# danijar/crafter

Hardware: AMD Instinct MI355X
Metric: env-steps/sec (whole node), random policy, 4096 envs (higher is better)
Workload: dtype u8/i32 (+f64 render filters)

## Files before the change

### __graft_entry__.py

```python
import pathlib
import sys

ROOT = pathlib.Path(__file__).resolve().parent
if str(ROOT) not in sys.path:
  sys.path.insert(0, str(ROOT))


def build():
  from crafter_amd import build as hip_build
  path = hip_build.build()
  print(f'[build] {path}')
  from oracle import noise
  print(f'[build] {noise.build()}')
  from tests.hostsim import build as hostsim_build
  print(f'[build] {hostsim_build.build()}')
  from tests.hostsim import symbolic_build
  print(f'[build] {symbolic_build.build()}')
  from tests.hostsim import final_build
  print(f'[build] {final_build.build()}')
  from tests.hostsim import levels_build
  print(f'[build] {levels_build.build()}')
  from tests.hostsim import subset_build
  print(f'[build] {subset_build.build()}')
  import crafter_amd
  from crafter_amd import lib
  lib.load()
  print('[build] crafter_amd imported, libcrafter_hip.so loaded, ABI', lib.load().crafter_abi_version())


def smoke():
  import numpy as np
  import torch
  from crafter_amd import BatchedEnv
  from oracle.crafter_oracle import OracleEnv
  from tests.parity import assert_same
  assert torch.cuda.is_available(), 'smoke() needs a GPU'
  seeds = [1000, 1001, 1002, 1003]
  env = BatchedEnv(len(seeds), seeds=seeds, device='cuda:0', auto_reset=False, semantic=True)
  orcs = [OracleEnv(seed=s) for s in seeds]
  obs = env.reset().cpu().numpy()
  for i, o in enumerate(orcs):
    assert np.array_equal(obs[i], o.reset()), f'reset obs env {i}'
  rs = np.random.RandomState(0)
  for t in range(30):
    acts = rs.randint(0, 17, size=len(seeds)).astype(np.int32)
    obs, rew, done, info = env.step(torch.from_numpy(acts).to('cuda:0'))
    obs, rew, done = obs.cpu().numpy(), rew.cpu().numpy(), done.cpu().numpy()
    for i, o in enumerate(orcs):
      ob, r, d, _ = o.step(int(acts[i]))
      assert np.array_equal(obs[i], ob) and rew[i] == np.float32(r) and bool(done[i]) == bool(d), (t, i)
  for i, o in enumerate(orcs):
    assert_same(env.snapshot(i), o.snapshot(), f'smoke env {i}')
  env.check_errors()
  print(f'[smoke] ok: {len(seeds)} envs x 30 steps bit-exact vs oracle on {torch.cuda.get_device_name(0)}; '
        f'LDS/env {env.lds_bytes} B')

# ... 6 lines not shown
```

### crafter_amd/build.py

```python
import pathlib
import shutil
import subprocess

ROOT = pathlib.Path(__file__).resolve().parent
SRC = ROOT / 'csrc' / 'crafter_hip.hip'
SRC_ROLLOUT = ROOT / 'csrc' / 'crafter_rollout.hip'
SRC_SUBSET = ROOT / 'csrc' / 'crafter_subset.hip'
OUT = ROOT / '_lib' / 'libcrafter_hip.so'
FLAGS = ['--offload-arch=gfx950', '-O3', '-std=c++17', '-ffp-contract=off', '-fPIC', '-shared']
CFLAGS = [f for f in FLAGS if f != '-shared']
ROLLOUT_FLAGS = ['-mllvm', '-disable-machine-licm']


def sources():
  return ([SRC, SRC_ROLLOUT, SRC_SUBSET] + sorted((ROOT / 'csrc').glob('*.hpp')) + sorted((ROOT / 'csrc').glob('*.inc')) +
          [ROOT.parent / 'include' / 'crafter_hip.h', ROOT.parent / 'include' / 'crafter_hip_types.h'])


def source_hash():
  import hashlib
  h = hashlib.sha256()
  for p in sorted(sources(), key=lambda q: q.name):
    h.update(p.name.encode() + b'\0' + p.read_bytes() + b'\0')
  return h.hexdigest()[:16]
# ... 30 lines not shown
      print(' '.join(cmd))
    proc = subprocess.run(cmd, capture_output=True, text=True)
    if proc.returncode != 0:
      raise RuntimeError(f'hipcc (link) failed:\n{proc.stdout}\n{proc.stderr}')
  return target


if __name__ == '__main__':
  print(build(force=True, verbose=True))


def resource_usage():
  import re
  import tempfile
  hipcc = shutil.which('hipcc') or '/opt/rocm/bin/hipcc'
  text = ''
  with tempfile.TemporaryDirectory() as tmp:
    for src, extra in ((SRC, []), (SRC_ROLLOUT, ROLLOUT_FLAGS), (SRC_SUBSET, [])):
      cmd = [hipcc] + CFLAGS + extra + ['-Rpass-analysis=kernel-resource-usage', '-c', '-o', str(pathlib.Path(tmp) / 'x.o'), str(src)]
      proc = subprocess.run(cmd, capture_output=True, text=True)
      if proc.returncode != 0:
        raise RuntimeError(proc.stderr)
      text += proc.stderr
  out, cur = {}, None
  for line in text.splitlines():
    m = re.search(r'Function Name: (\S+)', line)
    if m:
      name = re.search(r'crafter_[a-z_]+_kernel', m.group(1))
      targ = re.search(r'crafter_[a-z_]+_kernelILi(\d+)E(?:Li(\d+)E)?(?:Li(\d+)E)?', m.group(1))
      args = ','.join(a for a in targ.groups() if a is not None) if targ else ''
      key = (name.group(0) + (f'<{args}>' if targ else '')) if name else m.group(1)
      cur = out.setdefault(key, {})
      continue
    for key, pat in (('vgprs', r'VGPRs: (\d+)'), ('scratch', r'ScratchSize \[bytes/lane\]: (\d+)'),
                     ('occupancy', r'Occupancy \[waves/SIMD\]: (\d+)'), ('vgpr_spill', r'VGPRs Spill: (\d+)')):
      m = re.search(pat, line)
      if m and cur is not None:
        cur[key] = int(m.group(1))
  return out
```

### crafter_amd/csrc/crafter_hip.hip

```cpp
#include <hip/hip_runtime.h>
#include <hip/hip_ext.h>
#include <stdio.h>
#include <stdlib.h>
#include <string.h>

#include <map>
#include <mutex>
#include <string>
#include <vector>

#include "../../include/crafter_hip.h"
#include "crafter_rollout.hpp"
#include "crafter_subset.hpp"
#include "dispatch_order.hpp"
#include "env_copy.hpp"
#include "env_kernels.hpp"
#include "env_levels.hpp"
#include "launch_plan.hpp"
#include "legal.hpp"
#include "symbolic.hpp"
#include "wave_gfx950.hpp"

using namespace crafter;

namespace {

constexpr int kResetThreads = 1024;
constexpr int kRequeueGrid = 256;
constexpr int kRequeueGridPooled = 8;
constexpr int kGenSeedThreads = 64;
constexpr int kGenClassifyThreads = 256;
constexpr int kGenResolveThreads = 64;
constexpr int kGenSerialGrid = 2048;
constexpr int kGenClassifyGridStep = 304;
constexpr int kGenClassifyGrid = 256;
constexpr int kDefaultGenPeriod = 16;
constexpr int kUnpooledStretch = 16;
constexpr int kGenRing = 8;
constexpr int kGenLag = 3;
constexpr int kGenStreams = 2;
constexpr int kMaxLds = 160 * 1024;

template <int LM, int GEO, int RUL>
#ifndef CRAFTER_BIG_WAVES
#define CRAFTER_BIG_WAVES 6
#endif
__global__ void __launch_bounds__(kStepThreads, LM == 0 ? CRAFTER_BIG_WAVES : 1)
crafter_step_kernel(Config cfg_in, TablePtrs tb, StatePtrs st, const int32_t* __restrict__ actions,
                    uint8_t* __restrict__ obs, float* __restrict__ reward, uint8_t* __restrict__ done,
                    StepCtl ctl) {
  extern __shared__ __attribute__((aligned(16))) uint8_t smem[];
  typedef WaveGfx950<kStepThreads> WS;
  WS w;
  const Config cfg = GEO == 1 ? with_default_geometry(cfg_in) : GEO == 2 ? with_default_view(cfg_in) : cfg_in;
  int env = (int)blockIdx.x;
  if (ctl.order_build) {
    if (env == 0) {
      build_order(cfg, tb, ctl.order_build, ctl.next_step, (uint32_t*)smem);
      return;
    }
    env -= 1;
    if (ctl.order) env = ctl.order[env];
  }
  if constexpr (GEO == 1)
    step_body<WS, LM, RUL, uint8_t>(w, smem, env, cfg, tb, st, actions, obs, reward, done, ctl);
// ... 131 lines not shown

#ifndef CRAFTER_CLASSIFY_WAVES
#define CRAFTER_CLASSIFY_WAVES 6
#endif
template <int GEO>
__global__ void __launch_bounds__(kGenClassifyThreads, GEO ? CRAFTER_CLASSIFY_WAVES : 1)
crafter_gen_classify_kernel(Config cfg_in, TablePtrs tb, StatePtrs st, int parity, int prio) {
  extern __shared__ __attribute__((aligned(16))) uint8_t smem[];
  WaveGfx950<kGenClassifyThreads>::set_priority(prio);
  const Config cfg = GEO ? with_default_geometry(cfg_in) : cfg_in;
  const int32_t* q = st.gen_q + (size_t)parity * gen_q_stride(cfg);
  int count = q[0];
  if (count > gen_q_capacity(cfg)) count = gen_q_capacity(cfg);
  WaveGfx950<kGenClassifyThreads> w;
  const int parts = gen_classify_parts(cfg);
  for (int item = (int)blockIdx.x; item < count * parts; item += (int)gridDim.x) {
    int k = item / parts;
    gen_classify_body(w, smem, q[4 + 2 * k], q[4 + 2 * k + 1], item - k * parts, parts, cfg, tb, st);
    __syncthreads();
  }
}

template <int GEO>
__global__ void __launch_bounds__(kGenResolveThreads)
crafter_gen_resolve_kernel(Config cfg_in, TablePtrs tb, StatePtrs st, int parity, uint32_t seq, int prio) {
  extern __shared__ __attribute__((aligned(16))) uint8_t smem[];
  WaveGfx950<kGenResolveThreads>::set_priority(prio);
  const Config cfg = GEO ? with_default_geometry(cfg_in) : cfg_in;
  const int32_t* q = st.gen_q + (size_t)parity * gen_q_stride(cfg);
  int count = q[0];
  if (count > gen_q_capacity(cfg)) count = gen_q_capacity(cfg);
  WaveGfx950<kGenResolveThreads> w;
  for (int k = (int)blockIdx.x; k < count; k += (int)gridDim.x) {
    gen_resolve_body(w, smem, q[4 + 2 * k], q[4 + 2 * k + 1], seq, cfg, tb, st);
    __syncthreads();
  }
}

#ifdef CRAFTER_PROBES
template <int BIG>
__global__ void __launch_bounds__(kStepThreads)
crafter_gen_occupy_kernel(int us, int items, uint32_t* sink) {
  extern __shared__ __attribute__((aligned(16))) uint8_t smem[];
  if (BIG) asm volatile("v_mov_b32 v111, 0" ::: "v111");
  for (int k = (int)blockIdx.x; k < items; k += (int)gridDim.x) {
    uint64_t t0 = wall_clock64();
    while ((long long)(wall_clock64() - t0) < (long long)us * 100) __builtin_amdgcn_s_sleep(32);
  }
  if (sink && threadIdx.x == 0 && smem[0] == 0xA5) sink[0] = 1;
}

template <int GEO>
__global__ void __launch_bounds__(kStepThreads)
crafter_gen_stamp_kernel(Config cfg_in, TablePtrs tb, StatePtrs st, int parity, uint32_t seq) {
  typedef WaveGfx950<kStepThreads> WS;
  const Config cfg = GEO ? with_default_geometry(cfg_in) : cfg_in;
  const int32_t* q = st.gen_q + (size_t)parity * gen_q_stride(cfg);
  int count = q[0];
  if (count > gen_q_capacity(cfg)) count = gen_q_capacity(cfg);
  const int cells = cfg.W * cfg.H, nch = cfg.nchunk_x * cfg.nchunk_y;
  for (int k = (int)blockIdx.x; k < count; k += (int)gridDim.x) {
    int env = q[4 + 2 * k], episode = q[4 + 2 * k + 1];
    size_t slot = pool_slot(cfg, env, episode), other = pool_slot(cfg, env, episode + 1);
    PoolHdr* h = st.pool_hdr + slot;
    bool skip = !gen_wanted<WS>(st, env, episode) || gen_done_already<WS>(cfg, st, env, episode);
    bool never = (WS::agent_load(&h->ready) >> 32) == 0;
    __syncthreads();
// ... 240 lines not shown
}

int32_t crafter_abi_version(void) { return 7; }

int crafter_create(const crafter_config* cfg, crafter_handle** out) {
  if (!cfg || !out) return fail(nullptr, "crafter_create: null argument");
  const Config& c = *cfg;
  if (c.num_envs < 1) return fail(nullptr, "crafter_create: num_envs < 1");
  if (c.W < 1 || c.H < 1 || c.W * c.H > 4 * 65536) return fail(nullptr, "crafter_create: bad area");
  if (c.max_objects < 2 || c.max_objects > 65535) return fail(nullptr, "crafter_create: bad max_objects");
  if (c.unit_x < 1 || c.unit_y < 1 || c.local_gw < 1 || c.local_gh < 1)
    return fail(nullptr, "crafter_create: bad view geometry");
  if (c.size_w < 1 || c.size_h < 1 || (long long)c.size_w * c.size_h > (1 << 22))
    return fail(nullptr, "crafter_create: bad image size (at most 2^22 pixels)");
  if (render_static_bytes(c) + sprite_rows_bytes(c) > kRenderStaticBound)
    return fail(nullptr, "crafter_create: image size too large for the renderer's LDS tables (width + height of the view in pixels)");
  int count = 0;
  hipError_t e = hipGetDeviceCount(&count);
  if (e != hipSuccess || count < 1)
    return fail(nullptr, "crafter_create: no HIP device visible (this library has no CPU path)");
  crafter_handle* h = new crafter_handle();
  h->cfg = c;
  if (const char* pad = probe_env("CRAFTER_LDS_PAD")) h->lds_pad = atoi(pad) > 0 ? atoi(pad) : 0;
  if (const char* v = probe_env("CRAFTER_ROLLOUT_ORDER")) h->rollout_order = atoi(v) != 0;
  if (const char* v = probe_env("CRAFTER_FOLD_MAIN_EVENT")) h->fold_main_event = atoi(v) != 0;
  if (const char* v = probe_env("CRAFTER_GEN_SERIAL_PRIO")) h->gen_serial_prio = atoi(v);
  if (const char* v = probe_env("CRAFTER_GEN_CLASSIFY_PRIO")) h->gen_classify_prio = atoi(v);
  if (const char* v = probe_env("CRAFTER_PROBE_FREE_GEN")) h->probe_free_gen = atoi(v);
  if (const char* v = probe_env("CRAFTER_PROBE_OCCUPY_LDS")) sscanf(v, "%d,%d,%d", &h->probe_lds[0], &h->probe_lds[1], &h->probe_lds[2]);
  if (const char* v = probe_env("CRAFTER_PROBE_OCCUPY_BIG")) h->probe_big = atoi(v);
  if (const char* v = probe_env("CRAFTER_PROBE_OCCUPY")) sscanf(v, "%d,%d,%d,%d", &h->probe_worlds, &h->probe_us[0], &h->probe_us[1], &h->probe_us[2]);
  if (const char* pad = probe_env("CRAFTER_ROLLOUT_LDS_PAD")) h->rollout_lds_pad = atoi(pad) > 0 ? atoi(pad) : 0;
  h->plan = launch_plan(c, false, h->lds_pad, h->rollout_lds_pad);
  h->gen_resolve_lds_bytes = gen_resolve_layout(c).total;
  if (const char* v = probe_env("CRAFTER_GEN_LAG")) h->gen_lag = atoi(v) >= 1 && atoi(v) <= kGenRing - 2 ? atoi(v) : kGenLag;
  if (const char* v = getenv("CRAFTER_SPLIT")) h->split = atoi(v) < 0 ? -1 : atoi(v) != 0 ? 1 : 0;
  if (const char* v = probe_env("CRAFTER_NOISE_AHEAD")) h->noise_ahead = atoi(v) != 0;
  if (const char* v = getenv("CRAFTER_STEP_WIDE")) h->wide = atoi(v) != 0 ? 1 : 0;
  if (const char* v = getenv("CRAFTER_STEP_EARLY")) h->early_frame = atoi(v) != 0 ? 1 : 0;
  if (const char* v = probe_env("CRAFTER_REQUEUE_GRID")) h->requeue_grid = atoi(v) >= 1 && atoi(v) <= kRequeueGrid ? atoi(v) : kRequeueGridPooled;
  if (!h->plan.maps_in_lds) h->classify_grid = 2 * kGenClassifyGrid;
  h->classify_grid_step = h->plan.gen_geo ? kGenClassifyGridStep : h->classify_grid;
  if (const char* v = probe_env("CRAFTER_GEN_CLASSIFY_GRID")) h->classify_grid = h->classify_grid_step = atoi(v) > 0 ? atoi(v) : h->classify_grid;
  if (h->plan.render_lds > kMaxLds) {
    std::string msg = "crafter_create: one environment needs " + std::to_string(h->plan.render_lds) +
                      " B of LDS (> 160 KiB): area / max_objects too large for the LDS-resident kernels";
    delete h;
    return fail(nullptr, msg);
  }
  if ((c.step_threads != 0 && c.step_threads != kStepThreads) || (c.reset_threads != 0 && c.reset_threads != kResetThreads)) {
    delete h;
    return fail(nullptr, "crafter_create: workgroup sizes are fixed in this build (step_threads 0 or " +
                             std::to_string(kStepThreads) + ", reset_threads 0 or " + std::to_string(kResetThreads) + ")");
  }
  if (h->plan.opt_in_lds) {
    std::vector<const void*> big;
#define CRAFTER_X(id, LM, GEO, RUL) \
    if constexpr (GEO != 1) big.push_back((const void*)crafter_step_kernel<LM, GEO, RUL>);
    CRAFTER_STEP_INSTANCES(CRAFTER_X)
#undef CRAFTER_X
    for (const void* f : {(const void*)crafter_reset_kernel, (const void*)crafter_gen_resolve_kernel<0>,
                          (const void*)crafter_requeue_reset_kernel, (const void*)crafter_requeue_final_kernel,
                          (const void*)crafter_render_kernel})
      big.push_back(f);
    hipError_t er = rollout_allow_lds(h->plan.render_lds);
    if (er != hipSuccess) {
      std::string msg = std::string("crafter_create: hipFuncSetAttribute(rollout kernels): ") + hipGetErrorString(er);
// ... 1015 lines not shown
```

### crafter_amd/csrc/env_kernels.hpp

```cpp
#pragma once
#include "env_core.hpp"
#include "render.hpp"
#include "symbolic.hpp"
#include "worldgen.hpp"

namespace crafter {

__host__ __device__ inline bool is_default_geometry(const Config& c) {
  return c.W == 64 && c.H == 64 && c.view_w == 9 && c.view_h == 9 && c.size_w == 64 && c.size_h == 64 && c.unit_x == 7 &&
         c.unit_y == 7 && c.local_gw == 9 && c.local_gh == 7 && c.item_gw == 9 && c.item_gh == 2 && c.border_x == 0 &&
         c.border_y == 0 && c.icon_w == 5 && c.icon_h == 5 && c.digit_w == 4 && c.digit_h == 4 && c.max_objects == 256 &&
         c.nchunk_x == 6 && c.nchunk_y == 6 && c.update_dist == 18;
}
__device__ __forceinline__ Config with_default_geometry(Config c) {
  c.W = 64; c.H = 64; c.view_w = 9; c.view_h = 9; c.size_w = 64; c.size_h = 64; c.unit_x = 7; c.unit_y = 7;
  c.local_gw = 9; c.local_gh = 7; c.item_gw = 9; c.item_gh = 2; c.border_x = 0; c.border_y = 0; c.icon_w = 5; c.icon_h = 5;
  c.digit_w = 4; c.digit_h = 4; c.max_objects = 256; c.nchunk_x = 6; c.nchunk_y = 6; c.update_dist = 18;
  return c;
}

__host__ __device__ inline bool is_default_view(const Config& c) {
  return c.view_w == 9 && c.view_h == 9 && c.size_w == 64 && c.size_h == 64 && c.unit_x == 7 && c.unit_y == 7 && c.local_gw == 9 &&
         c.local_gh == 7 && c.item_gw == 9 && c.item_gh == 2 && c.border_x == 0 && c.border_y == 0 && c.icon_w == 5 && c.icon_h == 5 &&
         c.digit_w == 4 && c.digit_h == 4 && c.update_dist == 18;
// ... 1323 lines not shown
    for (int base = 64 * w.wave_index(); base < per; base += 64 * W::num_waves()) {
      uint64_t m = w.ballot(base, per, [&](int k) { return (state[k] & 15) != WorldGen<W>::NK_DONE; });
      if (!m) continue;
      uint32_t at = 0;
      if (w.lane() == 0) at = w.lds_fetch_add(count, (uint32_t)__builtin_popcountll(m));
      at = (uint32_t)W::uni((int)at);
      w.lanes(base, per, [&](int k, int lane) {
        if ((m >> lane) & 1ull) items[at + __builtin_popcountll(m & ((1ull << lane) - 1ull))] = (uint16_t)k;
      });
    }
    w.sync();
    int n = (int)*count;
    if (n == 0) break;
    GEN_COUNT(14);
    w.block_for(n, [&](int j) {
      int k = items[j];
      int i = first + k;
      int x = i / cfg.H, y = i - x * cfg.H;
      int stt = state[k];
      double v = WorldGen<W>::classify_lookup(sx, stt, x, y);
      uint8_t code = 0;
      int nxt = WorldGen<W>::classify_advance(ids, stt, v, code);
      state[k] = (uint8_t)nxt;
      if ((nxt & 15) == WorldGen<W>::NK_DONE) codes[i] = code;
    });
    w.sync();
  }
  GEN_STAMP(9);
  GEN_COUNT(15);
}

__host__ __device__ inline int gen_classify_lds_bytes(const Config&) { return kGenClassifyTables + 3 * kGenClassifyCells + 16; }

struct GenResolveLayout {
  int mat, objs, mt, wg, rec, rules, chunk_order, chunk_seen, census, scratch, total;
};
__host__ __device__ inline GenResolveLayout gen_resolve_layout(const Config& c) {
  GenResolveLayout G;
  int cells = c.W * c.H, nch = c.nchunk_x * c.nchunk_y;
  int o = 0;
  G.mat = lds_layout(c).maps_in_lds ? o : -1;
  if (G.mat >= 0) o += align16(cells);
  G.objs = G.mat >= 0 ? o : -1;
  if (G.objs >= 0) o += 16 * c.max_objects;
  G.mt = o;           o += align16(4 * MT_N);
  G.wg = o;           o += align16(WG_LDS_BYTES);
  G.rec = o;          o += align16((int)sizeof(EnvRec));
  G.rules = o;        o += CRAFTER_RULES_HEAD_BYTES;
  G.chunk_order = o;  o += align16(2 * nch);
  G.chunk_seen = o;   o += align16(nch);
  G.census = o;       o += align16(20 * nch);
  G.scratch = o;      o += 16;
  G.total = o;
  return G;
}

template <class W>
__device__ __forceinline__ void gen_resolve_body(W& w, uint8_t* smem, int env, int episode, uint32_t seq, const Config& cfg,
                                        const TablePtrs& tb, const StatePtrs& st) {
  if (!gen_wanted<W>(st, env, episode) || gen_done_already<W>(cfg, st, env, episode)) {
    if (w.leader()) gen_retire<W>(cfg, st, env, episode);
    return;
  }
  GenResolveLayout G = gen_resolve_layout(cfg);
  w.scratch = (uint32_t*)(smem + G.scratch);
  GEN_T0
  int cells = cfg.W * cfg.H;
  int nch = cfg.nchunk_x * cfg.nchunk_y;
  size_t slot = pool_slot(cfg, env, episode);
  Env<W> e(w, cfg, tb, smem + G.rules);
  e.g_mat = st.pool_mat + slot * cells;
  e.g_objmap = nullptr;
  e.objmap = nullptr;
  e.mat = G.mat >= 0 ? smem + G.mat : e.g_mat;
  e.objs = G.objs >= 0 ? (Obj*)(smem + G.objs) : st.pool_objs + slot * cfg.max_objects;
  e.mt = (uint32_t*)(smem + G.mt);
  e.rec = (EnvRec*)(smem + G.rec);
  e.chunk_order = (uint16_t*)(smem + G.chunk_order);
  e.chunk_seen = smem + G.chunk_seen;
  e.census = (int32_t*)(smem + G.census);
  {
    const uint32_t* src = (const uint32_t*)tb.rules;
    uint32_t* dst = (uint32_t*)&e.R;
    w.block_for(CRAFTER_RULES_HEAD_BYTES / 4, [&](int i) { dst[i] = src[i]; });
  }
  if (e.mat != e.g_mat) {
    if (cells % 16 == 0) {
      const uint4* src = (const uint4*)e.g_mat;
      uint4* dst = (uint4*)e.mat;
      w.block_for(cells / 16, [&](int i) { dst[i] = src[i]; });
    } else {
      w.block_for(cells, [&](int i) { e.mat[i] = e.g_mat[i]; });
    }
  }
  const uint32_t* gmt = st.pool_mt + slot * MT_N;
  w.block_for(MT_N, [&](int i) { e.mt[i] = gmt[i]; });
  w.block_for(nch, [&](int i) { e.chunk_seen[i] = 0; e.chunk_order[i] = 0; });
  e.clear_creature_counts();
  if (w.leader()) {
    e.rec->status = 0;
    e.rec->nchunks_seen = 0;
    Obj z;
    z.type = T_NONE; z.health = 0; z.fx = 0; z.fy = 0; z.x = 0; z.y = 0; z.aux = 0; z.pad = 0;
    e.objs[0] = z;
  }
  e.mt_pos = st.pool_hdr[slot].mt_pos;
  e.nobj = 1;
  e.dirty_slots = 0;
  e.rng_invalidate();
  w.sync();
  WorldGen<W> wg(e, smem + G.wg);
  int px = cfg.W / 2, py = cfg.H / 2;
  GEN_STAMP(16);
  if (w.wave0()) {
    e.obj_add(T_PLAYER, px, py, 0, 0, 1, 0);
    wg.window_open();
    GEN_STAMP(17);
    wg.resolve_materials(cells);
    GEN_STAMP(18);
    wg.place_creatures(cells, px, py);
    GEN_STAMP(19);
  }
  w.sync();
  share_registers(e);
  w.block_for(cells, [&](int i) {
    uint8_t m = (uint8_t)(e.mat[i] & WG_MAT_MASK);
    e.mat[i] = m;
    e.g_mat[i] = m;
  });
  w.sync();
  GEN_STAMP(20);
  e.recount_space();
  GEN_STAMP(21);
  int32_t* gcs = st.pool_census + slot * nch * 5;
  w.block_for(nch * 5, [&](int i) { gcs[i] = e.census[i]; });
  uint4* gob = (uint4*)(st.pool_objs + slot * cfg.max_objects);
  const uint4* lob = (const uint4*)e.objs;
  if (lob != gob) w.block_for(e.nobj, [&](int i) { gob[i] = lob[i]; });
  uint32_t* gmt_out = st.pool_mt + slot * MT_N;
  w.block_for(MT_N, [&](int i) { gmt_out[i] = e.mt[i]; });
  uint16_t* gco = st.pool_chunk_order + slot * nch;
  w.block_for(nch, [&](int i) { gco[i] = e.chunk_order[i]; });
  w.sync();
  if (w.leader()) {
    PoolHdr* h = st.pool_hdr + slot;
    h->mt_pos = e.mt_pos;
    h->nobj = e.nobj;
    h->nchunks_seen = e.rec->nchunks_seen;
    h->pad = (int32_t)e.rec->status;
    W::agent_store(&h->ready, ((uint64_t)seq << 32) | (uint32_t)episode);
    gen_retire<W>(cfg, st, env, episode);
  }
  GEN_STAMP(22);
  GEN_COUNT(31);
}

template <class W>
__device__ __forceinline__ void render_body(W& w, uint8_t* smem, int env, const Config& cfg, const TablePtrs& tb,
                                   const StatePtrs& st, uint8_t* out) {
  LdsLayout L = lds_layout(cfg);
  w.scratch = (uint32_t*)(smem + L.scratch);
  Env<W> e(w, cfg, tb, smem + L.rules);
  bind_lds(e, smem, L, st, env);
  RenderTarget rt = obs_target<W>(cfg, tb, out, env);
  Renderer<W> r(e, rt, smem + L.render, (uint32_t*)(smem + L.mtb), L.frame_bytes ? smem + L.frame : nullptr);
  if (out != nullptr) r.preload();
  load_env(e, st, env, 1);
  r.render(out != nullptr);
  w.sync();
  store_env(e, st, env, !L.frame_over_objs);
}

struct FinalOut {
// ... 71 lines not shown
```

### crafter_amd/csrc/wave_gfx950.hpp

```cpp
#pragma once
#include <hip/hip_runtime.h>

#include "mt19937.hpp"

namespace crafter {

__device__ __forceinline__ static void mt_wave_sync() {
  __builtin_amdgcn_fence(__ATOMIC_ACQ_REL, "wavefront");
  __builtin_amdgcn_wave_barrier();
}

template <int TEE>
__device__ __attribute__((noinline)) static void mt_twist_lds_impl(uint32_t* mt, uint32_t* tee) {
#if defined(__HIP_DEVICE_COMPILE__)
  __builtin_assume(__builtin_amdgcn_is_shared(mt));
#endif
  const int l = threadIdx.x & 63;
  uint32_t cur[4], nxt[4], far[4];
#pragma unroll
  for (int k = 0; k < 4; k++) {
    int i = l + 64 * k;
    if (i < 227) {
      cur[k] = mt[i];
      nxt[k] = mt[i + 1];
// ... 102 lines not shown
    int i = l + 64 * k;
    if (i < 227) {
      mt[i] = a[k];
      mt[227 + i] = b[k];
      tee[i] = a[k];
      tee[227 + i] = b[k];
    }
  }
#pragma unroll
  for (int k = 0; k < 3; k++) {
    int i = 454 + l + 64 * k;
    if (i < 623) {
      mt[i] = c[k];
      tee[i] = c[k];
    }
  }
  if (l == 0) {
    mt[623] = last;
    tee[623] = last;
  }
  mt_wave_sync();
}

template <int NT, int FRESH = 0, int EARLY = 0>
struct WaveGfx950 {
  static_assert(NT % 64 == 0 && NT >= 64, "whole waves");
  uint32_t* scratch;
  static constexpr bool kEarlyFrame = EARLY != 0 && NT > 64;
  static constexpr bool kConcurrentWaves = true;
  static constexpr int kDrawingWaves = NT > 64 ? NT / 64 - 1 : 1;
  __device__ __forceinline__ void spin_until(const uint32_t* p, uint32_t value) const {
    while (__hip_atomic_load(p, __ATOMIC_RELAXED, __HIP_MEMORY_SCOPE_WORKGROUP) < value) __builtin_amdgcn_s_sleep(2);
    __builtin_amdgcn_fence(__ATOMIC_ACQUIRE, "workgroup");
  }
  uint32_t tid_ = threadIdx.x;
  __device__ __forceinline__ uint32_t tx() const {
    if constexpr (FRESH != 0) {
      __builtin_assume(tid_ < (uint32_t)NT);
      return tid_;
    } else {
      return threadIdx.x;
    }
  }
  __device__ __forceinline__ void refresh() {
    if constexpr (FRESH != 0) asm volatile("" : "+v"(tid_));
  }
  __device__ __forceinline__ static void assume_lds(const void* p) {
#if defined(__HIP_DEVICE_COMPILE__)
    __builtin_assume(__builtin_amdgcn_is_shared(p));
#else
    (void)p;
#endif
  }

  __device__ __forceinline__ static float fdiv(float a, float b) { return __fdiv_rn(a, b); }
  __device__ __forceinline__ static int uni(int v) { return __builtin_amdgcn_readfirstlane(v); }
  __device__ __forceinline__ static int mul24(int a, int b) { return __mul24(a, b); }
  __device__ __forceinline__ static uint32_t mulhi24(uint32_t a, uint32_t b) {
    uint32_t r;
    asm("v_mul_hi_u32_u24 %0, %1, %2" : "=v"(r) : "v"(a), "v"(b));
    return r;
  }

  __device__ __forceinline__ static int opaque(int v) {
    asm volatile("" : "+s"(v));
    return v;
// ... 265 lines not shown
```

### crafter_amd/csrc/worldgen.hpp

```cpp
#pragma once
#include <math.h>

#include "env_core.hpp"
#include "simplex.hpp"

namespace crafter {

enum : uint8_t {
  WG_MAT_MASK = 0x0F,
  WG_TREE = 0x10,
  WG_TUNNEL = 0x40,
  WG_PENDING = 0x80,
};

constexpr int WG_TABLES_AT = 1024 + 4 * MT_N;
constexpr int WG_LDS_BYTES = WG_TABLES_AT + kSimplexLdsBytes;

struct DD {
  double hi, lo;
};
__device__ __forceinline__ DD dd_two_sum(double a, double b) {
  double s = a + b, bb = s - a;
  return {s, (a - (s - bb)) + (b - bb)};
}
// ... 21 lines not shown
                   {1.0, 0.0},
                   {0.5, 0.0},
                   {0x1.5555555555555p-3, 0x1.5555555555555p-57},
                   {0x1.5555555555555p-5, 0x1.5555555555555p-59},
                   {0x1.1111111111111p-7, 0x1.1111111111111p-63},
                   {0x1.6c16c16c16c17p-10, -0x1.f49f49f49f49fp-65},
                   {0x1.a01a01a01a01ap-13, 0x1.a01a01a01a01ap-73},
                   {0x1.a01a01a01a01ap-16, 0x1.a01a01a01a01ap-76}};
  double k = __builtin_rint(x * INV_LN2);
  double a = x - k * L1;
  DD p2 = dd_two_prod(k, L2);
  DD st = dd_two_sum(a, -p2.hi);
  double t = (st.lo - p2.lo) - k * L3;
  DD r = dd_quick_two_sum(st.hi, t);
  r.hi *= 0.00390625;
  r.lo *= 0.00390625;
  DD acc = C[8];
#pragma unroll
  for (int n = 7; n >= 0; n--) acc = dd_add(dd_mul(acc, r), C[n]);
#pragma unroll
  for (int i = 0; i < 8; i++) acc = dd_mul(acc, acc);
  double out = __builtin_ldexp(acc.hi, (int)k);
  DD one = dd_two_sum(1.0, x);
  double half_up = one.hi < 1.0 ? 0x1p-54 : 0x1p-53;
  uint64_t up;
  __builtin_memcpy(&up, &one.hi, 8);
  up += 1;
  double above;
  __builtin_memcpy(&above, &up, 8);
  double tiny = one.lo == half_up ? above : one.hi;
  return __builtin_fabs(x) <= 0x1p-52 ? tiny : out;
}

template <class W, class S = uint16_t>
struct WorldGen {
  Env<W, S>& e;
  uint8_t* perm;
  uint8_t* pg3;
  uint8_t* source;
  uint8_t* ridx;
  SimplexLds* tab;
  uint32_t* mtb;

  __device__ __forceinline__ WorldGen(Env<W, S>& env, uint8_t* lds) : e(env) {
    perm = lds;
    pg3 = lds + 256;
    source = lds + 512;
    ridx = lds + 768;
    tab = (SimplexLds*)(lds + WG_TABLES_AT);
    mtb = (uint32_t*)(lds + 1024);
  }

  __device__ __forceinline__ void seed_simplex(int64_t seed) {
    e.w.block_for(256, [&](int i) { ridx[i] = (uint8_t)simplex_shuffle_index(seed, i); });
    e.w.sync();
    e.w.block_for(256, [&](int i) { source[i] = (uint8_t)i; });
    e.w.sync();
    if (e.w.leader()) {
      const uint32_t* r4 = (const uint32_t*)ridx;
      uint32_t next = r4[63];
      for (int g = 63; g >= 0; g--) {
        uint32_t rr = next;
        next = r4[g > 0 ? g - 1 : 0];
#pragma unroll
        for (int k = 3; k >= 0; k--) {
          int i = 4 * g + k;
          int r = (int)((rr >> (8 * k)) & 0xFFu);
// ... 117 lines not shown
        if (v > 0.15 && (flags & NF_M30)) { code = R.path; return NK_DONE; }
        return NK_TUNH | flags;
      case NK_TUNH:
        if (v > 0.4) { code = (uint8_t)(R.path | WG_TUNNEL); return NK_DONE; }
        return NK_TUNV | flags;
      case NK_TUNV:
        if (v > 0.4) { code = (uint8_t)(R.path | WG_TUNNEL); return NK_DONE; }
        return NK_C1 | flags;
      case NK_C1:
        return NK_C2 | flags | (v > 0 ? NF_A : 0);
      case NK_C2: {
        flags |= (v > 0.4 ? NF_B : 0);
        if (flags & NF_M30) return NK_C4 | flags;
        v = 0.0;
      }
      case NK_C4: {
        int c1 = (flags & NF_A) != 0, c2 = (flags & NF_B) != 0, c3 = (flags & NF_M18) != 0;
        int c4 = (kind == NK_C4) && v > 0.35;
        code = !(c1 | c2 | c3) ? (c4 ? R.lava : R.stone) : (uint8_t)(WG_PENDING | c1 | (c2 << 1) | (c3 << 2) | (c4 << 3));
        return NK_DONE;
      }
      case NK_SAND:
        if (v > -0.2) { code = R.sand; return NK_DONE; }
        if (flags & NF_A) { code = R.water; return NK_DONE; }
        return NK_TREE;
      default:
        code = v > 0 ? (uint8_t)(WG_PENDING | WG_TREE) : R.grass;
        return NK_DONE;
    }
  }

  __device__ __forceinline__ void window_open() {
    e.rng_invalidate();
    if (e.mt_pos >= MT_N) {
      e.w.mt_twist(e.mt);
      e.mt_pos = 0;
    }
    e.w.wave_for(MT_N, [&](int i) { mtb[i] = e.mt[i]; });
    e.w.wsync();
    e.w.mt_twist(mtb);
  }
  __device__ __forceinline__ uint32_t wword(int k) const {
    int idx = e.mt_pos + k;
    return idx < MT_N ? e.mt[idx] : mtb[idx - MT_N];
  }
  __device__ __forceinline__ double wdouble(int d) const { return mt_double(mt_temper(wword(2 * d)), mt_temper(wword(2 * d + 1))); }
  __device__ __forceinline__ void advance(int nwords) {
    e.mt_pos += nwords;
    if (e.mt_pos >= MT_N) {
      e.w.wave_for(MT_N, [&](int i) { e.mt[i] = mtb[i]; });
      e.w.wsync();
      e.w.mt_twist(mtb);
      e.mt_pos -= MT_N;
    }
  }

  __device__ __forceinline__ static int draws_of(int code) {
    return (code & WG_TREE) ? 1 : __builtin_popcount(code & 7);
  }

  struct DrawWindow {
    uint64_t lo[4], hi[4];
    int p;
  };
  template <int NTHR>
  __device__ __forceinline__ void eval_chunk(int first, const double (&thr)[NTHR], uint64_t (&m)[4]) {
    W& w = e.w;
    w.lane_set(1, 0, 64, [&](int l, int) -> uint32_t {
      double d = wdouble(first + l);
      uint32_t bits = 0;
#pragma unroll
      for (int k = 0; k < NTHR; k++) bits |= (d > thr[k]) ? (1u << k) : 0u;
      return bits;
    });
#pragma unroll
    for (int k = 0; k < 4; k++) m[k] = k < NTHR ? W::uni64(w.lane_ballot(1, 1u << k)) : 0ull;
  }
  template <int NTHR>
  __device__ __forceinline__ void window_begin(DrawWindow& dw, const double (&thr)[NTHR]) {
    dw.p = 0;
    eval_chunk(0, thr, dw.lo);
    eval_chunk(64, thr, dw.hi);
    window_deal<NTHR>(dw);
  }
  template <int NTHR>
  __device__ __forceinline__ void window_roll(DrawWindow& dw, const double (&thr)[NTHR]) {
    if (dw.p >= 64) {
      advance(128);
#pragma unroll
      for (int k = 0; k < 4; k++) dw.lo[k] = dw.hi[k];
      eval_chunk(64, thr, dw.hi);
      dw.p -= 64;
      window_deal<NTHR>(dw);
    }
  }
  __device__ __forceinline__ void window_end(DrawWindow& dw) { advance(2 * dw.p); }
  __device__ __forceinline__ static uint32_t wbit(const DrawWindow& dw, int t, int pos) {
    uint64_t m = (pos & 64) ? dw.hi[t] : dw.lo[t];
    uint32_t half = (pos & 32) ? (uint32_t)(m >> 32) : (uint32_t)m;
    return (half >> (pos & 31)) & 1u;
  }

  __device__ __forceinline__ static uint32_t wword(const DrawWindow& dw, int t, int i) {
    uint64_t lo = dw.lo[t], hi = dw.hi[t];
    switch (i) {
      case 0: return (uint32_t)(lo << 16);
      case 1: return (uint32_t)(lo >> 16);
      case 2: return (uint32_t)((lo >> 48) | (hi << 16));
      case 3: return (uint32_t)(hi >> 16);
      case 4: return (uint32_t)(hi >> 48);
      default: return 0u;
    }
  }
  template <int NTHR>
  __device__ __forceinline__ void window_deal(const DrawWindow& dw) {
    W& w = e.w;
#pragma unroll
    for (int t = 0; t < NTHR; t++) w.lane_set(5 + t, 0, 64, [&](int, int l) -> uint32_t { return wword(dw, t, l); });
  }
  __device__ __forceinline__ uint32_t wfield(int t, int end, int l) const {
    uint32_t s = (uint32_t)(end + 1);
    int i = (int)(s >> 5);
    uint32_t lo = e.w.lane_fetch(5 + t, i, l), hi = e.w.lane_fetch(5 + t, i + 1, l);
    return (uint32_t)((((uint64_t)hi << 32) | lo) >> (s & 31u)) & 0xFFFFu;
  }
  __device__ __forceinline__ static uint64_t lanes_below(int n) { return n >= 64 ? ~0ull : ((1ull << n) - 1ull); }

  template <int NTHR>
  __device__ __forceinline__ uint64_t chain_round(const DrawWindow& dw, uint64_t active) {
// ... 50 lines not shown
  }
  __device__ __forceinline__ int count_used(uint64_t commit) {
    W& w = e.w;
    uint64_t u0 = w.lane_ballot(1, 1u << 8) & commit;
    uint64_t u1 = w.lane_ballot(1, 1u << 9) & commit;
    return __builtin_popcountll(u0) + 2 * __builtin_popcountll(u1);
  }

  static constexpr int kListCap = (kSimplexLdsBytes / 2) & ~63;
  __device__ __forceinline__ uint16_t* draw_list() const { return (uint16_t*)tab; }
  template <class F>
  __device__ __forceinline__ int build_draw_list(int& from, int cells, F links_of) {
    W& w = e.w;
    uint16_t* list = draw_list();
    const int first = from;
    int count = 0;
    while (from < cells && count + 64 <= kListCap && from - first < 65536 - 64) {
      uint64_t m = W::uni64(w.ballot(from, cells, [&](int i) { return links_of(i) != 0u; }));
      if (m) {
        w.lanes(from, cells, [&](int i, int l) {
          if ((m >> l) & 1ull) list[count + __builtin_popcountll(m & ((1ull << l) - 1ull))] = (uint16_t)(i - first);
        });
        count += __builtin_popcountll(m);
      }
      from += 64;
    }
    w.wsync();
    return count;
  }

  __device__ __forceinline__ void resolve_materials(int cells) {
    const Rules& R = e.R;
    W& w = e.w;
    const double thr[4] = {0.85, 0.75, 0.994, 0.8};
    DrawWindow dw;
    window_begin(dw, thr);
    auto links_of = [&](int i) -> uint32_t {
      int code = e.mat[i];
      if (!(code & WG_PENDING)) return 0u;
      return (code & WG_TREE) ? 8u : (uint32_t)((code & 7) | ((code & 8) << 1));
    };
    const uint16_t* list = draw_list();
    for (int from = 0; from < cells;) {
      const int first = from;
      const int count = build_draw_list(from, cells, links_of);
      for (int lb = 0; lb < count; lb += 64) {
        w.lane_set(2, lb, count, [&](int k, int) -> uint32_t { return (uint32_t)(first + list[k]); });
        w.lane_set(0, lb, count, [&](int, int l) -> uint32_t { return links_of((int)w.lane_get(2, l)); });
        uint64_t active = lanes_below(count - lb);
        while (active) {
          uint64_t commit = chain_round<4>(dw, active);
          w.lanes(lb, count, [&](int, int l) {
            if (!((commit >> l) & 1ull)) return;
            uint32_t links = w.lane_get(0, l), hit = w.lane_get(1, l) & 0xFFu;
            int m = (links & 8u) ? (hit ? R.mat_tree : R.mat_grass)
                    : hit == 1 ? R.mat_coal : hit == 2 ? R.mat_iron : hit == 3 ? R.mat_diamond : (links & 16u) ? R.mat_lava : R.mat_stone;
            e.mat[w.lane_get(2, l)] = (uint8_t)m;
          });
          w.wsync();
          dw.p += count_used(commit);
          active &= ~commit;
          window_roll(dw, thr);
        }
      }
    }
    window_end(dw);
  }

  __device__ __forceinline__ void place_creatures(int cells, int px, int py) {
    const Config& c = e.cfg;
    const Rules& R = e.R;
    W& w = e.w;
    const double thr[3] = {0.985, 0.993, 0.95};
    DrawWindow dw;
    window_begin(dw, thr);
    for (int base = 0; base < cells; base += 64) {
      w.lane_set(0, base, cells, [&](int i, int) -> uint32_t {
        int code = e.mat[i];
        int mat = code & WG_MAT_MASK;
        if (!((R.walkable_mask >> mat) & 1u)) return 0u;
        int x = i / c.H, y = i - x * c.H;
        int d2 = (x - px) * (x - px) + (y - py) * (y - py);
        uint32_t g = (d2 > 9 && mat == R.mat_grass);
        uint32_t z = (d2 > 100);
        uint32_t sk = (mat == R.mat_path && (code & WG_TUNNEL) != 0);
        return g | (z << 1) | (sk << 2);
      });
      uint64_t active = W::uni64(w.lane_ballot(0, 7u));
      while (active) {
        uint64_t commit = chain_round<3>(dw, active);
        uint64_t born = W::uni64(w.lane_ballot(1, 0xFFu)) & commit;
        while (born) {
          int l = __builtin_ctzll(born);
          born &= born - 1;
          int i = base + l;
          int x = i / c.H, y = i - x * c.H;
          int hit = (int)(w.lane_read(1, l) & 0xFF);
          int type = hit == 1 ? T_COW : hit == 2 ? T_ZOMBIE : T_SKELETON;
          e.obj_add(type, x, y, type == T_ZOMBIE ? 5 : 3, 0, 0, 0);
        }
        dw.p += count_used(commit);
        active &= ~commit;
        window_roll(dw, thr);
      }
    }
    window_end(dw);
// ... 81 lines not shown
```

Measured before the change: 66.54 million.

## Split world-gen resolve into producer/consumer waves with an LDS random-draw ring

The gen-resolve kernel now runs with 128 threads. A second wave continuously twists the Mersenne Twister state and evaluates threshold bitmasks for upcoming 128-word chunks, posting them into a small LDS ring. The first wave consumes these masks for material resolution and creature placement, so RNG generation overlaps with the serial draw logic instead of being interleaved with it. In exchange it adds LDS spin-wait synchronisation, a modular stream buffer over the MT state, and relocated object storage in LDS, which could reduce occupancy or add spin overhead.

```diff
diff --git a/__graft_entry__.py b/__graft_entry__.py
--- a/__graft_entry__.py
+++ b/__graft_entry__.py
@@ -22,6 +22,8 @@
   print(f'[build] {levels_build.build()}')
   from tests.hostsim import subset_build
   print(f'[build] {subset_build.build()}')
+  from tests.hostsim import resolve_ring_build
+  print(f'[build] {resolve_ring_build.build()}')
   import crafter_amd
   from crafter_amd import lib
   lib.load()
diff --git a/crafter_amd/build.py b/crafter_amd/build.py
--- a/crafter_amd/build.py
+++ b/crafter_amd/build.py
@@ -86,8 +86,9 @@
       key = (name.group(0) + (f'<{args}>' if targ else '')) if name else m.group(1)
       cur = out.setdefault(key, {})
       continue
-    for key, pat in (('vgprs', r'VGPRs: (\d+)'), ('scratch', r'ScratchSize \[bytes/lane\]: (\d+)'),
-                     ('occupancy', r'Occupancy \[waves/SIMD\]: (\d+)'), ('vgpr_spill', r'VGPRs Spill: (\d+)')):
+    for key, pat in (('vgprs', r' VGPRs: (\d+)'), ('scratch', r'ScratchSize \[bytes/lane\]: (\d+)'),
+                     ('occupancy', r'Occupancy \[waves/SIMD\]: (\d+)'), ('vgpr_spill', r'VGPRs Spill: (\d+)'),
+                     ('sgprs', r'TotalSGPRs: (\d+)'), ('lds', r'LDS Size \[bytes/block\]: (\d+)')):
       m = re.search(pat, line)
       if m and cur is not None:
         cur[key] = int(m.group(1))
diff --git a/crafter_amd/csrc/crafter_hip.hip b/crafter_amd/csrc/crafter_hip.hip
--- a/crafter_amd/csrc/crafter_hip.hip
+++ b/crafter_amd/csrc/crafter_hip.hip
@@ -30,7 +30,7 @@
 constexpr int kRequeueGridPooled = 8;
 constexpr int kGenSeedThreads = 64;
 constexpr int kGenClassifyThreads = 256;
-constexpr int kGenResolveThreads = 64;
+constexpr int kGenResolveThreads = 128;
 constexpr int kGenSerialGrid = 2048;
 constexpr int kGenClassifyGridStep = 304;
 constexpr int kGenClassifyGrid = 256;
@@ -228,7 +228,7 @@
   if (count > gen_q_capacity(cfg)) count = gen_q_capacity(cfg);
   WaveGfx950<kGenResolveThreads> w;
   for (int k = (int)blockIdx.x; k < count; k += (int)gridDim.x) {
-    gen_resolve_body(w, smem, q[4 + 2 * k], q[4 + 2 * k + 1], seq, cfg, tb, st);
+    gen_resolve_body<kDrawRing>(w, smem, q[4 + 2 * k], q[4 + 2 * k + 1], seq, cfg, tb, st);
     __syncthreads();
   }
 }
@@ -535,7 +535,7 @@
   if (const char* v = probe_env("CRAFTER_PROBE_OCCUPY")) sscanf(v, "%d,%d,%d,%d", &h->probe_worlds, &h->probe_us[0], &h->probe_us[1], &h->probe_us[2]);
   if (const char* pad = probe_env("CRAFTER_ROLLOUT_LDS_PAD")) h->rollout_lds_pad = atoi(pad) > 0 ? atoi(pad) : 0;
   h->plan = launch_plan(c, false, h->lds_pad, h->rollout_lds_pad);
-  h->gen_resolve_lds_bytes = gen_resolve_layout(c).total;
+  h->gen_resolve_lds_bytes = gen_resolve_layout(c, kDrawRing).total;
   if (const char* v = probe_env("CRAFTER_GEN_LAG")) h->gen_lag = atoi(v) >= 1 && atoi(v) <= kGenRing - 2 ? atoi(v) : kGenLag;
   if (const char* v = getenv("CRAFTER_SPLIT")) h->split = atoi(v) < 0 ? -1 : atoi(v) != 0 ? 1 : 0;
   if (const char* v = probe_env("CRAFTER_NOISE_AHEAD")) h->noise_ahead = atoi(v) != 0;
diff --git a/crafter_amd/csrc/env_kernels.hpp b/crafter_amd/csrc/env_kernels.hpp
--- a/crafter_amd/csrc/env_kernels.hpp
+++ b/crafter_amd/csrc/env_kernels.hpp
@@ -1379,16 +1379,17 @@
 
 __host__ __device__ inline int gen_classify_lds_bytes(const Config&) { return kGenClassifyTables + 3 * kGenClassifyCells + 16; }
 
+constexpr int kDrawRing = 4;
 struct GenResolveLayout {
-  int mat, objs, mt, wg, rec, rules, chunk_order, chunk_seen, census, scratch, total;
+  int mat, objs, mt, wg, rec, rules, chunk_order, chunk_seen, census, scratch, ring, total;
 };
-__host__ __device__ inline GenResolveLayout gen_resolve_layout(const Config& c) {
+__host__ __device__ inline GenResolveLayout gen_resolve_layout(const Config& c, int ring = 0) {
   GenResolveLayout G;
   int cells = c.W * c.H, nch = c.nchunk_x * c.nchunk_y;
   int o = 0;
   G.mat = lds_layout(c).maps_in_lds ? o : -1;
   if (G.mat >= 0) o += align16(cells);
-  G.objs = G.mat >= 0 ? o : -1;
+  G.objs = G.mat >= 0 && ring == 0 ? o : -1;
   if (G.objs >= 0) o += 16 * c.max_objects;
   G.mt = o;           o += align16(4 * MT_N);
   G.wg = o;           o += align16(WG_LDS_BYTES);
@@ -1398,18 +1399,21 @@
   G.chunk_seen = o;   o += align16(nch);
   G.census = o;       o += align16(20 * nch);
   G.scratch = o;      o += 16;
+  G.ring = o;         o += ring > 0 ? 64 * ring + 16 : 0;
   G.total = o;
   return G;
 }
 
-template <class W>
+template <int RING = 0, class W>
 __device__ __forceinline__ void gen_resolve_body(W& w, uint8_t* smem, int env, int episode, uint32_t seq, const Config& cfg,
                                         const TablePtrs& tb, const StatePtrs& st) {
   if (!gen_wanted<W>(st, env, episode) || gen_done_already<W>(cfg, st, env, episode)) {
     if (w.leader()) gen_retire<W>(cfg, st, env, episode);
     return;
   }
-  GenResolveLayout G = gen_resolve_layout(cfg);
+  GenResolveLayout G = gen_resolve_layout(cfg, RING);
+  using Gen = WorldGen<W, uint16_t, RING>;
+  static_assert(RING == 0 || 4 * Gen::kStreamWords <= (4 * MT_N + 15) / 16 * 16 + WG_TABLES_AT, "the stream buffer spans e.mt .. WorldGen::mtb");
   w.scratch = (uint32_t*)(smem + G.scratch);
   GEN_T0
   int cells = cfg.W * cfg.H;
@@ -1450,16 +1454,20 @@
     Obj z;
     z.type = T_NONE; z.health = 0; z.fx = 0; z.fy = 0; z.x = 0; z.y = 0; z.aux = 0; z.pad = 0;
     e.objs[0] = z;
+    if constexpr (RING > 0) {
+      uint32_t* ctl = (uint32_t*)(smem + G.ring + 64 * RING);
+      ctl[0] = ctl[1] = ctl[2] = ctl[3] = 0;
+    }
   }
   e.mt_pos = st.pool_hdr[slot].mt_pos;
   e.nobj = 1;
   e.dirty_slots = 0;
   e.rng_invalidate();
   w.sync();
-  WorldGen<W> wg(e, smem + G.wg);
+  Gen wg(e, smem + G.wg);
   int px = cfg.W / 2, py = cfg.H / 2;
   GEN_STAMP(16);
-  if (w.wave0()) {
+  auto draws = [&] {
     e.obj_add(T_PLAYER, px, py, 0, 0, 1, 0);
     wg.window_open();
     GEN_STAMP(17);
@@ -1467,8 +1475,15 @@
     GEN_STAMP(18);
     wg.place_creatures(cells, px, py);
     GEN_STAMP(19);
-  }
-  w.sync();
+  };
+  if constexpr (RING > 0) {
+    wg.ring_bind(smem + G.ring);
+    w.wave_pair([&] { draws(); wg.ring_finish(); }, [&] { wg.ring_produce(); });
+  } else if (w.wave0()) {
+    draws();
+  }
+  w.sync();
+  if constexpr (RING > 0) wg.ring_close();
   share_registers(e);
   w.block_for(cells, [&](int i) {
     uint8_t m = (uint8_t)(e.mat[i] & WG_MAT_MASK);
@@ -1485,7 +1500,7 @@
   const uint4* lob = (const uint4*)e.objs;
   if (lob != gob) w.block_for(e.nobj, [&](int i) { gob[i] = lob[i]; });
   uint32_t* gmt_out = st.pool_mt + slot * MT_N;
-  w.block_for(MT_N, [&](int i) { gmt_out[i] = e.mt[i]; });
+  w.block_for(MT_N, [&](int i) { gmt_out[i] = wg.state_word(i); });
   uint16_t* gco = st.pool_chunk_order + slot * nch;
   w.block_for(nch, [&](int i) { gco[i] = e.chunk_order[i]; });
   w.sync();
diff --git a/crafter_amd/csrc/wave_gfx950.hpp b/crafter_amd/csrc/wave_gfx950.hpp
--- a/crafter_amd/csrc/wave_gfx950.hpp
+++ b/crafter_amd/csrc/wave_gfx950.hpp
@@ -158,6 +158,20 @@
   __device__ __forceinline__ void spin_until(const uint32_t* p, uint32_t value) const {
     while (__hip_atomic_load(p, __ATOMIC_RELAXED, __HIP_MEMORY_SCOPE_WORKGROUP) < value) __builtin_amdgcn_s_sleep(2);
     __builtin_amdgcn_fence(__ATOMIC_ACQUIRE, "workgroup");
+  }
+  __device__ __forceinline__ void lds_post(uint32_t* p, uint32_t v) const {
+    __builtin_amdgcn_fence(__ATOMIC_RELEASE, "workgroup");
+    __hip_atomic_store(p, v, __ATOMIC_RELAXED, __HIP_MEMORY_SCOPE_WORKGROUP);
+  }
+  __device__ __forceinline__ uint32_t lds_peek(const uint32_t* p) const {
+    uint32_t v = __hip_atomic_load(p, __ATOMIC_RELAXED, __HIP_MEMORY_SCOPE_WORKGROUP);
+    __builtin_amdgcn_fence(__ATOMIC_ACQUIRE, "workgroup");
+    return (uint32_t)uni((int)v);
+  }
+  template <class A, class B>
+  __device__ __forceinline__ void wave_pair(A a, B b) const {
+    if (uni((int)(tx() < 64))) a();
+    else b();
   }
   uint32_t tid_ = threadIdx.x;
   __device__ __forceinline__ uint32_t tx() const {
diff --git a/crafter_amd/csrc/worldgen.hpp b/crafter_amd/csrc/worldgen.hpp
--- a/crafter_amd/csrc/worldgen.hpp
+++ b/crafter_amd/csrc/worldgen.hpp
@@ -77,7 +77,10 @@
   return __builtin_fabs(x) <= 0x1p-52 ? tiny : out;
 }
 
-template <class W, class S = uint16_t>
+#define WG_MATERIAL_THRESHOLDS 0.85, 0.75, 0.994, 0.8
+#define WG_CREATURE_THRESHOLDS 0.985, 0.993, 0.95
+
+template <class W, class S = uint16_t, int RING = 0>
 struct WorldGen {
   Env<W, S>& e;
   uint8_t* perm;
@@ -261,6 +264,7 @@
 
   __device__ __forceinline__ void window_open() {
     e.rng_invalidate();
+    if constexpr (RING > 0) return;
     if (e.mt_pos >= MT_N) {
       e.w.mt_twist(e.mt);
       e.mt_pos = 0;
@@ -307,6 +311,13 @@
   }
   template <int NTHR>
   __device__ __forceinline__ void window_begin(DrawWindow& dw, const double (&thr)[NTHR]) {
+    if constexpr (RING > 0) {
+      dw.p = rp;
+      ring_take<NTHR>(rk, dw.lo);
+      ring_take<NTHR>(rk + 1, dw.hi);
+      window_deal<NTHR>(dw);
+      return;
+    }
     dw.p = 0;
     eval_chunk(0, thr, dw.lo);
     eval_chunk(64, thr, dw.hi);
@@ -315,15 +326,104 @@
   template <int NTHR>
   __device__ __forceinline__ void window_roll(DrawWindow& dw, const double (&thr)[NTHR]) {
     if (dw.p >= 64) {
-      advance(128);
+      if constexpr (RING > 0) {
+        rk++;
+        e.w.lds_post(&rctl[1], (uint32_t)rk);
+      } else {
+        advance(128);
+      }
 #pragma unroll
       for (int k = 0; k < 4; k++) dw.lo[k] = dw.hi[k];
-      eval_chunk(64, thr, dw.hi);
+      if constexpr (RING > 0) ring_take<NTHR>(rk + 1, dw.hi);
+      else eval_chunk(64, thr, dw.hi);
       dw.p -= 64;
       window_deal<NTHR>(dw);
     }
   }
-  __device__ __forceinline__ void window_end(DrawWindow& dw) { advance(2 * dw.p); }
+  __device__ __forceinline__ void window_end(DrawWindow& dw) {
+    if constexpr (RING > 0) rp = dw.p;
+    else advance(2 * dw.p);
+  }
+
+  static constexpr int kStreamWords = MT_N + 128 * (RING + 1);
+  static constexpr int kRingBytes = RING > 0 ? 64 * RING + 16 : 0;
+  uint64_t* rrec = nullptr;
+  uint32_t* rctl = nullptr;
+  int rk = 0, rp = 0;
+  int rt = 0;
+  __device__ __forceinline__ void ring_bind(uint8_t* at) {
+    rrec = (uint64_t*)at;
+    rctl = (uint32_t*)(at + 64 * RING);
+  }
+  __device__ __forceinline__ static int sidx(int n) { return (int)((uint32_t)n % (uint32_t)kStreamWords); }
+  template <int NTHR>
+  __device__ __forceinline__ void ring_take(int chunk, uint64_t (&m)[4]) {
+    e.w.spin_until(&rctl[0], (uint32_t)chunk + 1u);
+    const uint64_t* r = rrec + 8 * (chunk % RING);
+    constexpr int at = NTHR == 4 ? 0 : 4;
+#pragma unroll
+    for (int k = 0; k < 4; k++) m[k] = k < NTHR ? W::uni64(r[at + k]) : 0ull;
+  }
+  __device__ __forceinline__ void ring_finish() {
+    e.w.lds_post(&rctl[2], (uint32_t)(e.mt_pos + 128 * rk + 2 * rp) + 1u);
+    e.w.lds_post(&rctl[1], 0xFFFFFFFFu);
+  }
+  __device__ __forceinline__ void ring_twist128(int E) {
+    uint32_t* s = e.mt;
+    e.w.lanes(E, E + 64, [&](int n, int) {
+      uint32_t c0 = s[sidx(n - MT_N)], n0 = s[sidx(n - MT_N + 1)], f0 = s[sidx(n - MT_N + MT_M)];
+      uint32_t c1 = s[sidx(n + 64 - MT_N)], n1 = s[sidx(n + 64 - MT_N + 1)], f1 = s[sidx(n + 64 - MT_N + MT_M)];
+      s[sidx(n)] = mt_twist_word(c0, n0, f0);
+      s[sidx(n + 64)] = mt_twist_word(c1, n1, f1);
+    });
+    e.w.wsync();
+  }
+  __device__ __forceinline__ void ring_produce() {
+    W& w = e.w;
+    const double thr[7] = {WG_MATERIAL_THRESHOLDS, WG_CREATURE_THRESHOLDS};
+    const uint32_t* s = e.mt;
+    const int pos0 = e.mt_pos;
+    int E = MT_N;
+    uint32_t fin = 0;
+    for (int c = 0;; c++) {
+      w.spin_until(&rctl[1], (uint32_t)(c >= RING ? c - RING + 1 : 0));
+      fin = w.lds_peek(&rctl[2]);
+      if (fin) break;
+      const int first = pos0 + 128 * c;
+      while (E < first + 128) {
+        ring_twist128(E);
+        E += 128;
+      }
+      w.lane_set(10, 0, 64, [&](int l, int) -> uint32_t {
+        double d = mt_double(mt_temper(s[sidx(first + 2 * l)]), mt_temper(s[sidx(first + 2 * l + 1)]));
+        uint32_t bits = 0;
+#pragma unroll
+        for (int k = 0; k < 7; k++) bits |= (d > thr[k]) ? (1u << k) : 0u;
+        return bits;
+      });
+      uint64_t* r = rrec + 8 * (c % RING);
+#pragma unroll
+      for (int k = 0; k < 7; k++) {
+        uint64_t m = W::uni64(w.lane_ballot(10, 1u << k));
+        w.lanes(0, 1, [&](int, int) { r[k] = m; });
+      }
+      w.lds_post(&rctl[0], (uint32_t)c + 1u);
+    }
+    const int t = (int)((fin - 1u) / (uint32_t)MT_N);
+    while (E < MT_N * (t + 1)) {
+      ring_twist128(E);
+      E += 128;
+    }
+  }
+  __device__ __forceinline__ void ring_close() {
+    uint32_t P = rctl[2] - 1u;
+    rt = (int)(P / (uint32_t)MT_N);
+    e.mt_pos = (int)(P - (uint32_t)rt * (uint32_t)MT_N);
+  }
+  __device__ __forceinline__ uint32_t state_word(int i) const {
+    if constexpr (RING > 0) return e.mt[sidx(MT_N * rt + i)];
+    else return e.mt[i];
+  }
   __device__ __forceinline__ static uint32_t wbit(const DrawWindow& dw, int t, int pos) {
     uint64_t m = (pos & 64) ? dw.hi[t] : dw.lo[t];
     uint32_t half = (pos & 32) ? (uint32_t)(m >> 32) : (uint32_t)m;
@@ -440,7 +540,7 @@
   __device__ __forceinline__ void resolve_materials(int cells) {
     const Rules& R = e.R;
     W& w = e.w;
-    const double thr[4] = {0.85, 0.75, 0.994, 0.8};
+    const double thr[4] = {WG_MATERIAL_THRESHOLDS};
     DrawWindow dw;
     window_begin(dw, thr);
     auto links_of = [&](int i) -> uint32_t {
@@ -479,7 +579,7 @@
     const Config& c = e.cfg;
     const Rules& R = e.R;
     W& w = e.w;
-    const double thr[3] = {0.985, 0.993, 0.95};
+    const double thr[3] = {WG_CREATURE_THRESHOLDS};
     DrawWindow dw;
     window_begin(dw, thr);
     for (int base = 0; base < cells; base += 64) {
```

After: 66.90 million, median of 6. No clear change (+0.5%).
